# European-XFEL/xFrame

Hardware: AMD Instinct MI355X
Metric: MTIP iterations/sec, 128 q-shells x L_max=32 (higher is better)
Workload: dtype f64 (complex128); 1 GPU; BASELINE config 4: 128 shells x L_max=32, grid 128x64x128, 8 restarts per GPU on 3 streams, tutorial schedule (HIO/SW/ER, ft_stab on), fused step; restarts_per_gpu=8, restarts_total=8, streams_per_gpu=3, engines_take_turns=True, parallelism=restart-sharded x1, step_mode=fused

## Files before the change

include/mtip_hip.h:

```cpp
#ifndef MTIP_HIP_H
#define MTIP_HIP_H

#include <stdint.h>

#ifdef __cplusplus
extern "C" {
#endif

typedef struct mtip_ctx mtip_ctx;
typedef struct { double re, im; } mtip_cdouble;

enum {
    MTIP_OK = 0,
    MTIP_EINVAL = -1,
    MTIP_ENODEV = -2,
    MTIP_EHIP = -3,
    MTIP_ENOMEM = -4,
    MTIP_ESTATE = -5
};

enum { MTIP_HIO = 0, MTIP_ER = 1, MTIP_HIO_NON_FXS = 2, MTIP_ER_NON_FXS = 3 };

enum { MTIP_PRE_NONE = 0, MTIP_PRE_SQUARE = 1 , MTIP_PRE_ABS = 2  };

// ... 166 lines not shown
int mtip2d_run(mtip2d_ctx* ctx, int method, int ft_stab, int n_steps, const double* betas, double* real_err);
int mtip2d_run_async(mtip2d_ctx* ctx, int method, int ft_stab, int n_steps, const double* betas);
int mtip2d_fetch_errors(mtip2d_ctx* ctx, int64_t first_step, int64_t n_steps, double* real_err);
int mtip2d_fetch_main_errors(mtip2d_ctx* ctx, int64_t first_step, int64_t n_steps, double* main_err);
int mtip2d_fetch_reciprocal_metrics(mtip2d_ctx* ctx, int64_t first_step, int64_t n_steps, double* deg2, double* l2);
int mtip2d_shrinkwrap(mtip2d_ctx* ctx, double sigma, double threshold, double error_limit, uint8_t* enforced);
int mtip2d_refresh_reciprocal_density(mtip2d_ctx* ctx);
int mtip2d_begin_sub_loop(mtip2d_ctx* ctx);
int mtip2d_select_best(mtip2d_ctx* ctx);
int mtip2d_select_best_where(mtip2d_ctx* ctx, const uint8_t* select);
int mtip2d_get_density(mtip2d_ctx* ctx, int batch, int which, mtip_cdouble* rho);
int mtip2d_get_reciprocal_density(mtip2d_ctx* ctx, int batch, int which, mtip_cdouble* F);
int mtip2d_get_support(mtip2d_ctx* ctx, int batch, int which, uint8_t* support);
int mtip2d_get_unknowns(mtip2d_ctx* ctx, int batch, mtip_cdouble* unknowns);
int mtip2d_get_best_error(mtip2d_ctx* ctx, double* best_error, int64_t* n_steps_done);
int mtip2d_synchronize(mtip2d_ctx* ctx);

int mtip_profile(mtip_ctx* ctx, int enable);
int mtip_profile_get(mtip_ctx* ctx, const char* name, double* total_ms, int64_t* launches);
int mtip_profile_reset(mtip_ctx* ctx);
int mtip_debug_jacobi_sweeps(mtip_ctx* ctx, int32_t* out);
int mtip_debug_chain_timing(mtip_ctx* ctx, int64_t* out);
int mtip_debug_hankel_tiles(mtip_ctx* ctx, int* ct, int* n_tiles, int* n_row_blocks);
int mtip_debug_projection_slots(mtip_ctx* ctx);
#define MTIP_POLAR_TIMING_SLOTS 40
int mtip_debug_polar_timing(mtip_ctx* ctx, int64_t* out);
int mtip_debug_spin(mtip_ctx* ctx, double microseconds);
int mtip_debug_check_jacobi_schedule(mtip_ctx* ctx, int k_max);

#ifdef __cplusplus
}
#endif
#endif
```

xframe_amd/csrc/k_hankel.hip:

```cpp
#include "mtip_internal.h"
#include <vector>

void launch_hankel_mfma(mtip_ctx* c, const double2* in, double2* out, int inverse);

void launch_hankel(mtip_ctx* c, const double2* in, double2* out, int inverse) {
    ProfScope ps(c, "hankel");
    launch_hankel_mfma(c, in, out, inverse);
}

__global__ void __launch_bounds__(256) k_coeff_diff(const double2* __restrict__ a, const double2* __restrict__ b,
                                                    double2* __restrict__ out, int N, int nlm, long long total) {
    const long long idx = (long long)blockIdx.x * blockDim.x + threadIdx.x;
    if (idx >= total) return;
    const int q = (int)((idx / nlm) % N);
    double2 v = a[idx];
    if (q > 0) v = csub(v, b[idx]);
    out[idx] = v;
}

void launch_coeff_diff(mtip_ctx* c, const double2* a, const double2* b, double2* out) {
    const long long total = (long long)c->B * c->N * c->nlm;
    hipLaunchKernelGGL(k_coeff_diff, dim3((unsigned)div_up(total, 256)), dim3(256), 0, c->stream, a, b, out, c->N,
                       c->nlm, total);
}

#define HT_CT_MAX 5
#define HT_KC 16
#define HT_ROWS 128
#define HT_WS (HT_ROWS + 16)
#define HT_THREADS 512
#define HT_NW (HT_KC * HT_ROWS / HT_THREADS)

struct HankelTile32 { int l, cflat0; };

template <int HT_CT, bool SUB>
__global__ void __launch_bounds__(HT_THREADS) k_hankel_tile(const double* __restrict__ in, double* __restrict__ out,
                                                            const double* __restrict__ W,
                                                            const HankelTile32* __restrict__ tiles, int N, int Np, int L,
                                                            int B, int poffs, double scale, int sign,
                                                            const double* __restrict__ in_sub, const uint8_t* __restrict__ sub_mask) {
    constexpr int HT_COLS = 16 * HT_CT;
    constexpr int HT_XS = HT_COLS + 16;
    constexpr int HT_NX = (HT_KC * HT_COLS + HT_THREADS - 1) / HT_THREADS;
    __shared__ double Ws[2][HT_KC][HT_WS];
    __shared__ double Xs[2][HT_KC][HT_XS];
    __shared__ double Ss[SUB ? 2 : 1][SUB ? HT_KC : 1][HT_XS];
    const int tid = threadIdx.x;
    const int wave = tid >> 6, lane = tid & 63;
    const HankelTile32 tinfo = tiles[blockIdx.x];
    const int l = tinfo.l;
    const int k_base = blockIdx.y * HT_ROWS;
    const int ncl = 4 * l + 2;
    const int nlm2 = 2 * (L + 1) * (L + 1);
    const double* Wl = W + (size_t)l * Np * N;
    const int wrow = tid >> 5, wcol = (tid & 31) * 4;
    int xrow[HT_NX], xc[HT_NX];
    size_t xoff[HT_NX];
    bool xok[HT_NX], xsub[HT_NX];
#pragma unroll
    for (int j = 0; j < HT_NX; ++j) {
        const int e = tid + j * HT_THREADS;
        xrow[j] = e / HT_COLS;
        xc[j] = e - xrow[j] * HT_COLS;
        const int cflat = tinfo.cflat0 + xc[j];
        xok[j] = xrow[j] < HT_KC && cflat < B * ncl;
        const int b = xok[j] ? cflat / ncl : 0;
        const int within = xok[j] ? cflat - b * ncl : 0;
        xoff[j] = (size_t)b * N * nlm2 + 2 * (size_t)l * l + within;
        xsub[j] = SUB && (sub_mask == nullptr || sub_mask[b] != 0);
    }
    double rw0[HT_NW], rx0[HT_NX], rw1[HT_NW], rx1[HT_NX];
    double rs0[SUB ? HT_NX : 1], rs1[SUB ? HT_NX : 1];
    auto request = [&](int p0, double (&rw)[HT_NW], double (&rx)[HT_NX], double (&rs)[SUB ? HT_NX : 1]) {
        const int p = p0 + wrow;
        const bool p_ok = p < Np;
        const double* wr = Wl + (size_t)(p_ok ? p : 0) * N + k_base + wcol;
#pragma unroll
        for (int j = 0; j < HT_NW; ++j) rw[j] = (p_ok && k_base + wcol + j < N) ? wr[j] : 0.0;
#pragma unroll
        for (int j = 0; j < HT_NX; ++j) {
            const bool ok = xok[j] && p0 + xrow[j] < Np;
            const size_t o = xoff[j] + (size_t)(p0 + xrow[j] + poffs) * nlm2;
            rx[j] = ok ? in[o] : 0.0;
            if (SUB) {
                rs[j] = (ok && xsub[j]) ? in_sub[o] : 0.0;
                rx[j] -= rs[j];
            }
        }
    };
    auto deposit = [&](int buf, const double (&rw)[HT_NW], const double (&rx)[HT_NX], const double (&rs)[SUB ? HT_NX : 1]) {
#pragma unroll
        for (int j = 0; j < HT_NW; ++j) Ws[buf][wrow][wcol + j] = rw[j];
#pragma unroll
        for (int j = 0; j < HT_NX; ++j)
            if (xrow[j] < HT_KC) {
                Xs[buf][xrow[j]][xc[j]] = rx[j];
                if (SUB) Ss[buf][xrow[j]][xc[j]] = rs[j];
            }
    };
    const int li = lane & 15, kk = lane >> 4;
    v4f64 acc[HT_CT];
#pragma unroll
    for (int t = 0; t < HT_CT; ++t) acc[t] = v4f64{0.0, 0.0, 0.0, 0.0};
    auto multiply = [&](int buf) {
#pragma unroll
        for (int s = 0; s < HT_KC / 4; ++s) {
            const double af = Ws[buf][4 * s + kk][wave * 16 + li];
#pragma unroll
            for (int t = 0; t < HT_CT; ++t) {
                const double bf = Xs[buf][4 * s + kk][16 * t + li];
                acc[t] = __builtin_amdgcn_mfma_f64_16x16x4f64(af, bf, acc[t], 0, 0, 0);
            }
            if (SUB && wave == 0 && k_base == 0) {
                const double a0 = li == 0 ? af : 0.0;
#pragma unroll
                for (int t = 0; t < HT_CT; ++t) {
                    const double sf = Ss[buf][4 * s + kk][16 * t + li];
                    acc[t] = __builtin_amdgcn_mfma_f64_16x16x4f64(a0, sf, acc[t], 0, 0, 0);
                }
            }
        }
    };
    const int n_chunks = (Np + HT_KC - 1) / HT_KC;
    request(0, rw0, rx0, rs0);
    deposit(0, rw0, rx0, rs0);
    if (n_chunks > 1) request(HT_KC, rw1, rx1, rs1);
    if (n_chunks > 2) request(2 * HT_KC, rw0, rx0, rs0);
    __syncthreads();
    for (int i = 0; i < n_chunks; i += 2) {
        multiply(0);
        if (i + 1 < n_chunks) deposit(1, rw1, rx1, rs1);
        __syncthreads();
        if (i + 3 < n_chunks) request((i + 3) * HT_KC, rw1, rx1, rs1);
        if (i + 1 >= n_chunks) break;
        multiply(1);
        if (i + 2 < n_chunks) deposit(0, rw0, rx0, rs0);
        __syncthreads();
        if (i + 4 < n_chunks) request((i + 4) * HT_KC, rw0, rx0, rs0);
    }
    int r = l & 3;
    if (sign < 0) r = (4 - r) & 3;
    const bool is_im = (li & 1) != 0;
#pragma unroll
    for (int t = 0; t < HT_CT; ++t) {
        const int cflat = tinfo.cflat0 + 16 * t + li;
        const bool col_ok = cflat < B * ncl;
        const int b = col_ok ? cflat / ncl : 0;
        const int within = col_ok ? cflat - b * ncl : 0;
        const size_t col_off = (size_t)b * N * nlm2 + 2 * (size_t)l * l + within;
#pragma unroll
        for (int j = 0; j < 4; ++j) {
            double v = acc[t][j] * scale;
            const double partner = __shfl_xor(v, 1, 64);
            double o;
            if (r == 0) o = v;
            else if (r == 2) o = -v;
            else if (r == 1) o = is_im ? partner : -partner;
            else o = is_im ? -partner : partner;
            const int k = k_base + wave * 16 + kk + 4 * j;
            if (col_ok && k < N) out[col_off + (size_t)k * nlm2] = o;
        }
    }
}

bool hankel_has_difference(const mtip_ctx* c) { return c->d_htiles32 != nullptr; }

int hankel_row_blocks(const mtip_ctx* c) { return div_up(c->N, HT_ROWS); }

void launch_hankel_mfma_sub(mtip_ctx* c, const double2* in, const double2* in_sub, double2* out, int inverse, const uint8_t* sub_mask) {
    const dim3 grid((unsigned)c->n_htiles32, (unsigned)hankel_row_blocks(c));
#define HT_LAUNCH(CT, SUBF)                                                                                                  \
    hipLaunchKernelGGL((k_hankel_tile<CT, SUBF>), grid, dim3(HT_THREADS), 0, c->stream, reinterpret_cast<const double*>(in), \
                       reinterpret_cast<double*>(out), (const double*)c->d_W, (const HankelTile32*)c->d_htiles32, c->N,      \
                       c->Np, c->L, c->B, c->cfg.hankel_trapz ? 1 : 0, inverse ? c->inv_scale : c->fwd_scale,                \
                       inverse ? +1 : -1, reinterpret_cast<const double*>(in_sub), sub_mask)
    if (in_sub != nullptr) {
        switch (c->htile_ct) {
            case 1: HT_LAUNCH(1, true); break;
            case 2: HT_LAUNCH(2, true); break;
            case 3: HT_LAUNCH(3, true); break;
            default: HT_LAUNCH(5, true); break;
        }
    } else {
        switch (c->htile_ct) {
            case 1: HT_LAUNCH(1, false); break;
            case 2: HT_LAUNCH(2, false); break;
            case 3: HT_LAUNCH(3, false); break;
            default: HT_LAUNCH(5, false); break;
        }
    }
#undef HT_LAUNCH
}

void launch_hankel_mfma(mtip_ctx* c, const double2* in, double2* out, int inverse) {
    launch_hankel_mfma_sub(c, in, nullptr, out, inverse);
}

int build_hankel_tiles(mtip_ctx* c) {
    std::vector<HankelTile32> t32;
    const int cts[4] = {5, 3, 2, 1};
    for (int ci = 0; ci < 4; ++ci) {
        t32.clear();
        c->htile_ct = cts[ci];
        for (int l = c->L; l >= 0; --l) {
            const int ncols = c->B * (4 * l + 2);
            for (int c0 = 0; c0 < ncols; c0 += 16 * cts[ci]) t32.push_back(HankelTile32{l, c0});
        }
        if (c->htile_force > 0 ? cts[ci] == c->htile_force : (int)t32.size() * hankel_row_blocks(c) * 5 >= c->n_cu * 4) break;
    }
    {
        const int X = 8;
        std::vector<std::vector<HankelTile32>> q(X);
        size_t i0 = 0;
        while (i0 < t32.size()) {
            size_t i1 = i0;
// ... 26 lines not shown
```

xframe_amd/csrc/mtip_api.hip:

```cpp
#include "mtip_internal.h"
#include <algorithm>
#include <cmath>
#include <cstdlib>
#include <cstring>

static thread_local std::string g_create_error;

#define CTX_CHECK(c)                       \
    do {                                   \
        if ((c) == nullptr) return MTIP_EINVAL; \
    } while (0)
#define FAIL(c, code, msg)      \
    do {                        \
        (c)->err = (msg);       \
        return (code);          \
    } while (0)

static int post_launch(mtip_ctx* c, const char* what) {
    hipError_t e = hipGetLastError();
    if (e != hipSuccess) {
        c->err = std::string(what) + ": " + hipGetErrorString(e);
        return MTIP_EHIP;
    }
    return MTIP_OK;
// ... 87 lines not shown
    auto A = [&](int r) { if (rc == MTIP_OK) rc = r; };
    if (hipStreamCreateWithFlags(&c->stream, hipStreamNonBlocking) != hipSuccess) A(MTIP_EHIP);
    {
        int ncu = 0;
        if (hipDeviceGetAttribute(&ncu, hipDeviceAttributeMultiprocessorCount, device) == hipSuccess && ncu > 0) c->n_cu = ncu;
    }
    (void)hipEventCreate(&c->ev0);
    (void)hipEventCreate(&c->ev1);
    A(dev_alloc(c, &c->d_cost, c->nt));
    A(dev_alloc(c, &c->d_gw, c->nt));
    A(dev_alloc(c, &c->d_P, (size_t)(L + 1) * (L + 2) / 2 * c->nt));
    A(dev_alloc(c, &c->d_poff, L + 2));
    c->npairs = (L + 1) * (L + 2) / 2;
    A(dev_alloc(c, &c->d_PT, (size_t)(c->nt / 2 + 1) * c->npairs));
    A(dev_alloc(c, &c->d_AB, (size_t)c->npairs + L + 1));
    A(dev_alloc(c, &c->d_lmtab, c->npairs));
    A(dev_alloc(c, &c->d_PTc, (size_t)(c->nt / 2 + 1) * 768));
    A(dev_alloc(c, &c->d_lmc, 768));
    if (const char* e = std::getenv("MTIP_DEG2_SIMPLE")) c->deg2_simple = std::atoi(e) != 0;
    if (const char* e = std::getenv("MTIP_HANKEL_CT")) {
        const int v = std::atoi(e);
        c->htile_force = (v == 1 || v == 2 || v == 3 || v == 5) ? v : 0;
    }
    if (rc == MTIP_OK) rc = build_hankel_tiles(c);
    A(dev_alloc(c, &c->d_twN, c->np));
    A(dev_alloc(c, &c->d_tw, c->np / 2));
    A(dev_alloc(c, &c->d_r, N));
    A(dev_alloc(c, &c->d_q, N));
    A(dev_alloc(c, &c->d_W, (size_t)(L + 1) * c->Np * N));
    c->kl.assign(L + 1, 0);
    c->used.assign(L + 1, 0);
    c->active.assign(L + 1, 0);
    c->voff.assign(L + 2, 0);
    c->xoff.assign(L + 2, 0);
    c->uoff.assign(L + 2, 0);
    c->have_V.assign(L + 1, 0);
    c->v_real.assign(L + 1, 1);
    c->psw = read_proj_switches();
    for (int l = 0; l <= L; ++l) {
        const int n = 2 * l + 1, k = std::min(n, N);
        c->kl[l] = k;
        c->voff[l + 1] = c->voff[l] + N * k;
        c->xoff[l + 1] = c->xoff[l] + k * n;
        c->uoff[l + 1] = c->uoff[l] + k * k;
    }
    c->vtot = c->voff[L + 1];
// ... 1085 lines not shown
    if (!c->d_polar_dbg) {
        int r = dev_alloc(c, &c->d_polar_dbg, n);
        if (r) return r;
        MTIP_HIP_CHECK(c, hipMemsetAsync(c->d_polar_dbg, 0, n * sizeof(long long), c->stream));
    }
    if (out) MTIP_HIP_CHECK(c, mtip_copy(c, out, c->d_polar_dbg, n * sizeof(long long), hipMemcpyDeviceToHost));
    return MTIP_OK;
}

int mtip_debug_chain_timing(mtip_ctx* c, int64_t* out) {
    CTX_CHECK(c);
    (void)hipSetDevice(c->device);
    const size_t n = (size_t)3 * c->B * c->N * MTIP_CHAIN_DBG_SLOTS;
    MTIP_HIP_CHECK(c, hipStreamSynchronize(c->stream));
    if (!c->d_chain_dbg) {
        int r = dev_alloc(c, &c->d_chain_dbg, n);
        if (r) return r;
        MTIP_HIP_CHECK(c, hipMemsetAsync(c->d_chain_dbg, 0, n * sizeof(long long), c->stream));
    }
    if (out) MTIP_HIP_CHECK(c, mtip_copy(c, out, c->d_chain_dbg, n * sizeof(long long), hipMemcpyDeviceToHost));
    return MTIP_OK;
}

int mtip_debug_check_jacobi_schedule(mtip_ctx* c, int k_max) {
    CTX_CHECK(c);
    if (k_max < 2 || k_max > 127) FAIL(c, MTIP_EINVAL, "k_max must be in [2, 127]");
    (void)hipSetDevice(c->device);
    MTIP_HIP_CHECK(c, hipStreamSynchronize(c->stream));
    const int r = build_jacobi_schedule(c, k_max);
    if (r != MTIP_OK) FAIL(c, r, "pairing schedule failed its verification");
    return MTIP_OK;
}

int mtip_profile_reset(mtip_ctx* c) {
    CTX_CHECK(c);
    prof_flush(c);
    c->prof_data.clear();
    return MTIP_OK;
}

}

void prof_flush(mtip_ctx* c) {
    if (c->prof_pending.empty()) {
        c->prof_next = 0;
        return;
// ... 15 lines not shown
```

xframe_amd/csrc/mtip_internal.h:

```cpp
#pragma once
#include <hip/hip_runtime.h>
#include <stdint.h>
#include <algorithm>
#include <map>
#include <string>
#include <type_traits>
#include <utility>
#include <vector>
#include "../../include/mtip_hip.h"

#ifndef MTIP_PIN_VGPRS4
#define MTIP_PIN_VGPRS4(a, b, c, d) asm volatile("" : "+v"(a), "+v"(b), "+v"(c), "+v"(d));
#endif
#ifndef MTIP_WAIT_LDS
#define MTIP_WAIT_LDS() asm volatile("s_waitcnt lgkmcnt(0)" ::: "memory")
#endif


#ifndef MTIP_WAVE_LDS_SYNC
#define MTIP_WAVE_LDS_SYNC()                        \
    do {                                            \
        asm volatile("" ::: "memory");              \
        __builtin_amdgcn_wave_barrier();            \
        asm volatile("" ::: "memory");              \
// ... 10 lines not shown
}
__device__ __forceinline__ double2 cadd(double2 a, double2 b) { return make_double2(a.x + b.x, a.y + b.y); }
__device__ __forceinline__ double2 csub(double2 a, double2 b) { return make_double2(a.x - b.x, a.y - b.y); }
__device__ __forceinline__ double2 cscale(double2 a, double s) { return make_double2(a.x * s, a.y * s); }
__device__ __forceinline__ double cabs2(double2 a) { return a.x * a.x + a.y * a.y; }
__device__ __forceinline__ int isqrt_lm(int lm) {
    int l = (int)sqrt((double)lm);
    while (l * l > lm) --l;
    while ((l + 1) * (l + 1) <= lm) ++l;
    return l;
}
__device__ __forceinline__ double2 cmul_ipow(double2 a, int l, int sign) {
    int r = l & 3;
    if (sign < 0) r = (4 - r) & 3;
    switch (r) {
        case 0: return a;
        case 1: return make_double2(-a.y, a.x);
        case 2: return make_double2(-a.x, -a.y);
        default: return make_double2(a.y, -a.x);
    }
}

#define MTIP_CHAIN_DBG_SLOTS 18
#define MTIP_POLAR_DBG_SLOTS MTIP_POLAR_TIMING_SLOTS
enum { SL_CUR = 0, SL_OUT = 1, SL_BEST = 2, SL_SUP = 3, SL_SUP_BEST = 4, SL_ENFORCE = 5, SL_HAS_ERR = 6, SL_HIST = 7, SL_N = 8 };

enum { RC_SUPPORT = 1, RC_VALUE_LO = 2, RC_VALUE_HI = 4, RC_LIMIT_IMAG = 8 };

struct RealParams {
    uint32_t flags, hio_flags;
    double lo, hi, imag_thr;
};

__device__ __forceinline__ double2 real_update_point(const RealParams& rp, int method, double beta, double2 w, double2 pv,
                                                     bool S, double2& P_out) {
    double2 P = w;
    uint32_t viol = 0;
    if (rp.flags & RC_SUPPORT) {
        if (!S) {
            P = make_double2(0.0, 0.0);
            viol |= RC_SUPPORT;
        }
    }
    if ((rp.flags & RC_VALUE_LO) && (rp.flags & RC_VALUE_HI)) {
        if (P.x < rp.lo) { P.x = rp.lo; viol |= RC_VALUE_LO; }
        if (P.x > rp.hi) { P.x = rp.hi; viol |= RC_VALUE_LO; }
// ... 186 lines not shown
    DevBuf<int> d_lmtab;
    int npairs = 0;
    ShtPlan sht;
    DevBuf<double2> d_twN;
    DevBuf<double2> d_tw;
    DevBuf<double> d_W;
    int n_cu = 256;
    JacobiSchedule js;
    uint32_t im_which = 0;
    DevBuf<uint8_t> d_im_zmask;
    DevBuf<double2> d_im_IIref, d_im_ccdref;
    DevBuf<double> d_rl2_wr, d_rl2_wt, d_rl2_part, d_rl2_hist;
    DevBuf<double> d_im_fq;
    DevBuf<double2> d_im_part;
    DevBuf<double> d_im_qq, d_im_ccdT, d_im_P, d_im_refavg, d_im_refw, d_im_hist;
    double im_ccd_inv_norm = 0.0;
    int so_order = -1;
    DevBuf<long long> d_polar_dbg;
    DevBuf<double2> d_c0n;
    DevBuf<long long> d_chain_dbg;
    bool c0n_valid = false;
    DevBuf<HankelTile32> d_htiles32;
    int htile_force = 0;
    int n_htiles32 = 0, htile_ct = 5;
    double fwd_scale = 0, inv_scale = 0;
    bool have_angular = false, have_radial = false, have_weights = false, have_support = false, have_errw = false;
    ProjSwitches psw;
    ProjPlan pp;
    std::vector<int> kl, used, active, voff, xoff, uoff;
    DevBuf<int> d_active;
    DevBuf<int> d_sweeps;
    std::vector<char> v_real;
    std::vector<double2> h_V;
    int vr = VR_NONE;
    long long proj_calls = 0;
    DevBuf<int> d_kl, d_used, d_voff, d_xoff, d_uoff;
    int vtot = 0, xtot = 0, utot = 0;
    DevBuf<double2> d_V;
    DevBuf<uint8_t> d_rmask;
    std::vector<char> have_V;
    double n_particles = 1.0;
    int deg2_enable = 0;
    DevBuf<double2> d_Bref;
    DevBuf<double> d_Bnorm;
    DevBuf<double> d_deg2_part;
    bool deg2_simple = false;
// ... 37 lines not shown

void plan_sht(mtip_ctx* c);
int launch_sht_forward(mtip_ctx* c, const double2* grid, double2* coeff, int prologue, int in_slot = -1);
struct InvEpilogue {
    int mode = EPI_STORE;
    const double2* F = nullptr;
    const double* fixed = nullptr;
    const double* shell_scale = nullptr;
    const double2* coeff_sub = nullptr;
    RealEpi real;
    int out_slot = -1;
};
int launch_sht_inverse(mtip_ctx* c, const double2* coeff, double2* grid, const InvEpilogue& epi);
void build_legendre_tables(mtip_ctx* c, const double* cos_theta);
int sht_no_kernel(mtip_ctx* c, const char* what, int epi_mode);
void launch_sht_forward_fused(mtip_ctx* c, const double2* grid, double2* coeff, int prologue, int in_slot);
int launch_sht_inverse_fused(mtip_ctx* c, const double2* coeff, double2* grid, const InvEpilogue& epi);
void launch_sht_forward_reg(mtip_ctx* c, const double2* grid, double2* coeff, int prologue, int in_slot);
int launch_sht_inverse_reg(mtip_ctx* c, const double2* coeff, double2* grid, const InvEpilogue& epi);
int launch_sht_chain(mtip_ctx* c, const double2* coeff, double2* grid, const InvEpilogue& epi, int prologue, double2* coeff_out);
void launch_hankel(mtip_ctx* c, const double2* in, double2* out, int inverse);
bool hankel_has_difference(const mtip_ctx* c);
void launch_hankel_mfma_sub(mtip_ctx* c, const double2* in, const double2* in_sub, double2* out, int inverse, const uint8_t* sub_mask = nullptr);
int build_jacobi_schedule(mtip_ctx* c, int kmax);
int jacobi_groups(int k);
int build_hankel_tiles(mtip_ctx* c);
int hankel_row_blocks(const mtip_ctx* c);
int launch_invariant_metrics(mtip_ctx* c, const double2* Ilm, long long step);
int launch_reciprocal_l2_metric(mtip_ctx* c, const double2* F, const double2* Fp, long long step);
void launch_deg2(mtip_ctx* c, const double2* Ilm, double2* Bl);
void launch_coeff_diff(mtip_ctx* c, const double2* a, const double2* b, double2* out);
int launch_project_coefficients(mtip_ctx* c, const double2* Ilm, double2* out, bool real_intensity = false);
void plan_projection(mtip_ctx* c);
void plan_rproj(mtip_ctx* c);
void invalidate_projection(mtip_ctx* c);
int launch_rproj(mtip_ctx* c, double2* coef);
int launch_apply_unknowns(mtip_ctx* c, const double2* Ilm, double2* out);
void launch_deg2_metric(mtip_ctx* c, const double2* Ilm, double* out );
void launch_real_update(mtip_ctx* c, const double2* rho_p, const double2* prev, const double2* rho_rt, double2* out,
                        int method, double beta, int use_slots);
void launch_finish_step(mtip_ctx* c, long long step_index, int nblk = 0);
void launch_abs_to_fixed(mtip_ctx* c);
void launch_modulus_plain(mtip_ctx* c, const double2* F, const double2* Inew, double2* out);
void launch_modulus_fixed_slots(mtip_ctx* c, const double2* F);
void launch_copy_to_slot(mtip_ctx* c, const double2* src, double2* dst_slots, int which);
void launch_sw_clamp(mtip_ctx* c, const double2* conv, double* tmp_real);
// ... 91 lines not shown
```

xframe_amd/fxs/_lib.py:

```python
import ctypes as C
import os

import numpy as np

os.environ.setdefault('GPU_MAX_HW_QUEUES', '8')

_HERE = os.path.dirname(os.path.abspath(__file__))
DEFAULT_LIB = os.path.join(os.path.dirname(_HERE), 'csrc', 'libmtip_hip.so')

c_double_p = C.POINTER(C.c_double)
c_u8_p = C.POINTER(C.c_uint8)
c_void = C.c_void_p


class MtipCfg(C.Structure):
    _fields_ = [('n_radial', C.c_int32), ('l_max', C.c_int32), ('n_theta', C.c_int32), ('n_phi', C.c_int32),
                ('n_batch', C.c_int32), ('hankel_trapz', C.c_int32), ('fused', C.c_int32), ('reserved', C.c_int32)]


class MtipCorrelateCfg(C.Structure):
    _fields_ = [('n_q', C.c_int32), ('n_phi', C.c_int32), ('n_q1', C.c_int32), ('n_q2', C.c_int32), ('filter_kind', C.c_int32),
                ('roi_lo', C.c_int32), ('roi_hi', C.c_int32), ('roi_filter', C.c_int32), ('roi_normalize', C.c_int32),
                ('shared_mask', C.c_int32), ('filter_k', C.c_double), ('roi_min', C.c_double), ('roi_max', C.c_double)]

# ... 113 lines not shown
    'mtip_op_so3_find_rotation': (C.c_int, [c_void, c_void, c_void, C.c_int, C.c_int, c_void, c_void, c_void]),
    'mtip_op_rotate_coefficients_grid': (C.c_int, [c_void, c_void, c_void, c_void, c_void, c_void]),
    'mtip_op_hermitian_eig': (C.c_int, [c_void, C.c_int, C.c_int, c_void, c_void, c_void]),
    'mtip_op_symmetric_eig': (C.c_int, [c_void, C.c_int, C.c_int, c_void, c_void, c_void]),
    'mtip_op_cc_to_deg2': (C.c_int, [c_void, C.c_int, C.c_int, C.c_int, C.c_int, C.c_int, C.c_uint32, c_void, c_void, c_void, c_void, c_void]),
    'mtip_correlate_create': (c_void, [c_void, C.POINTER(MtipCorrelateCfg), c_void, c_void, c_void]),
    'mtip_correlate_destroy': (None, [c_void]),
    'mtip_correlate_add': (C.c_int, [c_void, C.c_int, c_void, c_void]),
    'mtip_correlate_num_patterns': (C.c_int, [c_void]),
    'mtip_correlate_get_partial': (C.c_int, [c_void, c_void, c_void, c_void, c_void]),
    'mtip_correlate_merge': (C.c_int, [c_void, c_void, c_void, C.c_int, c_void, c_void]),
    'mtip_correlate_finalize': (C.c_int, [c_void, C.c_int, C.c_int, C.c_int, C.c_int, C.c_int, c_void, c_void]),
    'mtip_resample_create': (c_void, [c_void, C.POINTER(MtipResampleCfg), c_void, c_void, c_void, c_void]),
    'mtip_resample_destroy': (None, [c_void]),
    'mtip_resample_run': (C.c_int, [c_void, C.c_int, c_void, C.c_int, c_void, c_void, c_void, C.POINTER(C.c_int64)]),
    'mtip_correlate_add_detector': (C.c_int, [c_void, c_void, C.c_int, c_void, C.c_int, c_void, C.POINTER(C.c_int64)]),
    'mtip_profile': (C.c_int, [c_void, C.c_int]),
    'mtip_profile_get': (C.c_int, [c_void, C.c_char_p, C.POINTER(C.c_double), C.POINTER(C.c_int64)]),
    'mtip_profile_reset': (C.c_int, [c_void]),
    'mtip_debug_jacobi_sweeps': (C.c_int, [c_void, c_void]),
    'mtip_debug_projection_slots': (C.c_int, [c_void]),
    'mtip_debug_hankel_tiles': (C.c_int, [c_void, c_void, c_void, c_void]),
    'mtip_debug_chain_timing': (C.c_int, [c_void, c_void]),
    'mtip_debug_check_jacobi_schedule': (C.c_int, [c_void, C.c_int]),
    'mtip_debug_polar_timing': (C.c_int, [c_void, c_void]),
    'mtip_debug_spin': (C.c_int, [c_void, C.c_double]),
}

EXPORTED_SYMBOLS = tuple(_SIGNATURES)
_libs = {}


def load(path=None):
    path = os.path.abspath(path or DEFAULT_LIB)
    if path in _libs:
        return _libs[path]
    if not os.path.exists(path):
        raise MtipError(f'{path} not found: build it with `python -c "import __graft_entry__ as g; g.build()"` '
                        '(hipcc --offload-arch=gfx950). There is no CPU fallback.')
    try:
        import torch
    except ImportError:
        pass
    lib = C.CDLL(path)
    for name, (res, args) in _SIGNATURES.items():
        fn = getattr(lib, name)
# ... 24 lines not shown
```

xframe_amd/fxs/engine.py:

```python
import ctypes as C

import numpy as np

from . import _lib, hostsetup as hs
from .settings import reciprocity_coefficient, resolve

METHOD_ID = {'HIO': 0, 'ER': 1, 'HIO_non_FXS': 2, 'ER_non_FXS': 3}


class Engine:
    def __init__(self, settings=None, data=None, n_batch=1, device=0, fused=True, lib_path=None,
                 n_radial=None, l_max=None, max_q=None):
        self.lib = _lib.load(lib_path)
        self.device_index = int(device)
        self.emulated = hasattr(self.lib, 'mtip_emulated')
        opt = resolve(settings)
        self.opt = opt
        g = opt['grid']
        self.N = int(n_radial if n_radial is not None else g['n_radial_points'])
        self.L = int(l_max if l_max is not None else g['max_order'])
        self.kappa = float(reciprocity_coefficient(opt['fourier_transform']))
        self.mode = opt['fourier_transform']['type']
        if max_q is None:
            max_q = g['max_q']
# ... 602 lines not shown
    def profile_get(self, name):
        ms, n = C.c_double(0), C.c_int64(0)
        self._ck(self.lib.mtip_profile_get(self.ctx, name.encode(), C.byref(ms), C.byref(n)))
        return ms.value, n.value

    def debug_spin(self, microseconds):
        self._ck(self.lib.mtip_debug_spin(self.ctx, float(microseconds)))

    def jacobi_sweeps(self):
        out = np.zeros((self.B, self.L + 1), np.int32)
        self._ck(self.lib.mtip_debug_jacobi_sweeps(self.ctx, _lib.ptr(out)))
        return out & 0xff

    def jacobi_active_columns(self):
        out = np.zeros((self.B, self.L + 1), np.int32)
        self._ck(self.lib.mtip_debug_jacobi_sweeps(self.ctx, _lib.ptr(out)))
        return (out >> 8) & 0xffff

    def hankel_tiles(self):
        ct, nt, nr = C.c_int(0), C.c_int(0), C.c_int(0)
        self._ck(self.lib.mtip_debug_hankel_tiles(self.ctx, C.byref(ct), C.byref(nt), C.byref(nr)))
        return ct.value, nt.value, nr.value

    def projection_slots(self):
        n = self.lib.mtip_debug_projection_slots(self.ctx)
        if n < 0:
            self._ck(n)
        return int(n)

    def jacobi_closing_step(self):
        out = np.zeros((self.B, self.L + 1), np.int32)
        self._ck(self.lib.mtip_debug_jacobi_sweeps(self.ctx, _lib.ptr(out)))
        return (out >> 24) & 3

    @property
    def thetas(self):
        return self.theta

    @property
    def phis(self):
        return self.phi

    def ft(self, grid):
        return self.fourier_transform(grid)[0]

    def forward_l(self, grid):
# ... 106 lines not shown
```

Before: 17180 MTIP iterations/s.

## Pipeline Hankel MFMA tiles with async global-to-LDS loads and 3-stage buffering

Rewrites the Hankel tile kernel's main loop to use global_load_lds direct DMA into a dynamically sized multi-stage LDS ring (default 3 stages), with vmcnt-based waits instead of register staging and double-buffered syncthreads. It also XOR-swizzles the X tile layout to avoid bank conflicts and replaces the extra row-0 MFMA for the difference term with a masked subtract plus a scalar FMA chain. The aim is to hide global-load latency and cut register and LDS-store traffic. The cost is more LDS per block, which may reduce occupancy, plus more complex waitcnt logic. A timed debug variant and API hook are added.

Result: faster. 17470 MTIP iterations/s (median of 6 runs) (+1.7%).

```diff
diff --git a/include/mtip_hip.h b/include/mtip_hip.h
--- a/include/mtip_hip.h
+++ b/include/mtip_hip.h
@@ -212,6 +212,7 @@
 int mtip_debug_jacobi_sweeps(mtip_ctx* ctx, int32_t* out);
 int mtip_debug_chain_timing(mtip_ctx* ctx, int64_t* out);
 int mtip_debug_hankel_tiles(mtip_ctx* ctx, int* ct, int* n_tiles, int* n_row_blocks);
+int mtip_debug_hankel_timing(mtip_ctx* ctx, int difference, int inverse, int64_t* out);
 int mtip_debug_projection_slots(mtip_ctx* ctx);
 #define MTIP_POLAR_TIMING_SLOTS 40
 int mtip_debug_polar_timing(mtip_ctx* ctx, int64_t* out);
diff --git a/xframe_amd/csrc/k_hankel.hip b/xframe_amd/csrc/k_hankel.hip
--- a/xframe_amd/csrc/k_hankel.hip
+++ b/xframe_amd/csrc/k_hankel.hip
@@ -1,4 +1,5 @@
 #include "mtip_internal.h"
+#include <type_traits>
 #include <vector>
 
 void launch_hankel_mfma(mtip_ctx* c, const double2* in, double2* out, int inverse);
@@ -30,48 +31,101 @@
 #define HT_WS (HT_ROWS + 16)
 #define HT_THREADS 512
 #define HT_NW (HT_KC * HT_ROWS / HT_THREADS)
+#ifndef HT_NS
+#define HT_NS 3
+#endif
 
 struct HankelTile32 { int l, cflat0; };
 
 template <int HT_CT, bool SUB>
+struct HankelLds {
+    static constexpr int COLS = 16 * HT_CT;
+    static constexpr int W_STAGE = HT_KC * HT_WS;
+    static constexpr int X_STAGE = HT_KC * COLS;
+    static constexpr int STAGE = W_STAGE + (SUB ? 2 : 1) * X_STAGE;
+    static constexpr size_t BYTES = (size_t)HT_NS * STAGE * sizeof(double);
+};
+
+__device__ __forceinline__ void ht_dma16(const double* src, double* dst, int lane) {
+#if defined(__HIP_DEVICE_COMPILE__)
+    (void)lane;
+    __builtin_amdgcn_global_load_lds((const __attribute__((address_space(1))) void*)src,
+                                     (__attribute__((address_space(3))) void*)dst, 16, 0, 0);
+#else
+    dst[2 * lane] = src[0];
+    dst[2 * lane + 1] = src[1];
+#endif
+}
+template <int CNT>
+__device__ __forceinline__ void ht_wait_vm() {
+#if defined(__HIP_DEVICE_COMPILE__)
+    asm volatile("s_waitcnt vmcnt(%0)" ::"n"(CNT) : "memory");
+#endif
+}
+__device__ __forceinline__ void ht_barrier() {
+#if defined(__HIP_DEVICE_COMPILE__)
+    asm volatile("s_waitcnt lgkmcnt(0)" ::: "memory");
+    __builtin_amdgcn_s_barrier();
+    asm volatile("" ::: "memory");
+#else
+    __syncthreads();
+#endif
+}
+
+template <int HT_CT, bool SUB, bool ROW0_MFMA, bool TIMED>
 __global__ void __launch_bounds__(HT_THREADS) k_hankel_tile(const double* __restrict__ in, double* __restrict__ out,
                                                             const double* __restrict__ W,
                                                             const HankelTile32* __restrict__ tiles, int N, int Np, int L,
                                                             int B, int poffs, double scale, int sign,
-                                                            const double* __restrict__ in_sub, const uint8_t* __restrict__ sub_mask) {
-    constexpr int HT_COLS = 16 * HT_CT;
-    constexpr int HT_XS = HT_COLS + 16;
+                                                            const double* __restrict__ in_sub, const uint8_t* __restrict__ sub_mask,
+                                                            long long* __restrict__ dbg) {
+    using G = HankelLds<HT_CT, SUB>;
+    constexpr int HT_COLS = G::COLS;
     constexpr int HT_NX = (HT_KC * HT_COLS + HT_THREADS - 1) / HT_THREADS;
-    __shared__ double Ws[2][HT_KC][HT_WS];
-    __shared__ double Xs[2][HT_KC][HT_XS];
-    __shared__ double Ss[SUB ? 2 : 1][SUB ? HT_KC : 1][HT_XS];
+    constexpr bool DIRECT0 = SUB && !ROW0_MFMA;
+    constexpr int NQ = 2 * HT_CT;
+    constexpr int NXI = (NQ + 7) / 8;
+    constexpr int NHI = NQ % 8;
+    constexpr int NXL = NHI ? NXI - 1 : NXI;
+    HIP_DYNAMIC_SHARED(double, lds)
     const int tid = threadIdx.x;
-    const int wave = tid >> 6, lane = tid & 63;
+    const int lane = tid & 63;
+    const int wave = __builtin_amdgcn_readfirstlane(tid >> 6);
+    long long* tl = reinterpret_cast<long long*>(lds + HT_NS * G::STAGE);
+    auto stamp = [&](int slot) {
+        if constexpr (TIMED) {
+            if (wave == 0 || wave == 5) {
+                const long long t = clock64();
+                if (lane == 0) tl[(wave ? 1 : 0) * MTIP_HANKEL_DBG_SLOTS + slot] = t;
+            }
+        }
+    };
+    auto stamp_chunk = [&](int chunk, int what) {
+        if (chunk < MTIP_HANKEL_DBG_CHUNKS) stamp(2 + 4 * chunk + what);
+    };
+    if constexpr (TIMED) {
+        if (tid < 2 * MTIP_HANKEL_DBG_SLOTS) tl[tid] = 0;
+        __syncthreads();
+        stamp(0);
+    }
     const HankelTile32 tinfo = tiles[blockIdx.x];
     const int l = tinfo.l;
     const int k_base = blockIdx.y * HT_ROWS;
     const int ncl = 4 * l + 2;
     const int nlm2 = 2 * (L + 1) * (L + 1);
+    const int ncols = B * ncl;
     const double* Wl = W + (size_t)l * Np * N;
+    auto xs_idx = [](int r, int c) { return r * HT_COLS + ((HT_COLS % 32 == 0) ? (c ^ ((r & 1) << 4)) : c); };
     const int wrow = tid >> 5, wcol = (tid & 31) * 4;
     int xrow[HT_NX], xc[HT_NX];
-    size_t xoff[HT_NX];
-    bool xok[HT_NX], xsub[HT_NX];
 #pragma unroll
     for (int j = 0; j < HT_NX; ++j) {
         const int e = tid + j * HT_THREADS;
         xrow[j] = e / HT_COLS;
         xc[j] = e - xrow[j] * HT_COLS;
-        const int cflat = tinfo.cflat0 + xc[j];
-        xok[j] = xrow[j] < HT_KC && cflat < B * ncl;
-        const int b = xok[j] ? cflat / ncl : 0;
-        const int within = xok[j] ? cflat - b * ncl : 0;
-        xoff[j] = (size_t)b * N * nlm2 + 2 * (size_t)l * l + within;
-        xsub[j] = SUB && (sub_mask == nullptr || sub_mask[b] != 0);
-    }
-    double rw0[HT_NW], rx0[HT_NX], rw1[HT_NW], rx1[HT_NX];
-    double rs0[SUB ? HT_NX : 1], rs1[SUB ? HT_NX : 1];
-    auto request = [&](int p0, double (&rw)[HT_NW], double (&rx)[HT_NX], double (&rs)[SUB ? HT_NX : 1]) {
+    }
+    double rw[HT_NW], rx[HT_NX], rs[SUB ? HT_NX : 1];
+    auto request = [&](int p0) {
         const int p = p0 + wrow;
         const bool p_ok = p < Np;
         const double* wr = Wl + (size_t)(p_ok ? p : 0) * N + k_base + wcol;
@@ -79,72 +133,205 @@
         for (int j = 0; j < HT_NW; ++j) rw[j] = (p_ok && k_base + wcol + j < N) ? wr[j] : 0.0;
 #pragma unroll
         for (int j = 0; j < HT_NX; ++j) {
-            const bool ok = xok[j] && p0 + xrow[j] < Np;
-            const size_t o = xoff[j] + (size_t)(p0 + xrow[j] + poffs) * nlm2;
+            const int cflat = tinfo.cflat0 + xc[j];
+            const bool ok = xrow[j] < HT_KC && cflat < ncols && p0 + xrow[j] < Np;
+            const int b = ok ? cflat / ncl : 0;
+            const int within = ok ? cflat - b * ncl : 0;
+            const size_t o = (size_t)b * N * nlm2 + 2 * (size_t)l * l + within + (size_t)(p0 + xrow[j] + poffs) * nlm2;
             rx[j] = ok ? in[o] : 0.0;
-            if (SUB) {
-                rs[j] = (ok && xsub[j]) ? in_sub[o] : 0.0;
-                rx[j] -= rs[j];
-            }
+            if (SUB) rs[j] = (ok && (sub_mask == nullptr || sub_mask[b] != 0)) ? in_sub[o] : 0.0;
         }
     };
-    auto deposit = [&](int buf, const double (&rw)[HT_NW], const double (&rx)[HT_NX], const double (&rs)[SUB ? HT_NX : 1]) {
-#pragma unroll
-        for (int j = 0; j < HT_NW; ++j) Ws[buf][wrow][wcol + j] = rw[j];
+    auto deposit = [&](int st) {
+        double* ws = lds + st * G::STAGE;
+#pragma unroll
+        for (int j = 0; j < HT_NW; ++j) ws[wrow * HT_WS + wcol + j] = rw[j];
 #pragma unroll
         for (int j = 0; j < HT_NX; ++j)
             if (xrow[j] < HT_KC) {
-                Xs[buf][xrow[j]][xc[j]] = rx[j];
-                if (SUB) Ss[buf][xrow[j]][xc[j]] = rs[j];
+                ws[G::W_STAGE + xs_idx(xrow[j], xc[j])] = rx[j];
+                if (SUB) ws[G::W_STAGE + G::X_STAGE + xs_idx(xrow[j], xc[j])] = rs[j];
             }
     };
     const int li = lane & 15, kk = lane >> 4;
+    bool subf[HT_CT];
+#pragma unroll
+    for (int t = 0; t < HT_CT; ++t) {
+        const int cflat = tinfo.cflat0 + 16 * t + li;
+        const bool ok = SUB && cflat < ncols;
+        subf[t] = ok && (sub_mask == nullptr || sub_mask[ok ? cflat / ncl : 0] != 0);
+    }
+    int subm[HT_CT];
+#pragma unroll
+    for (int t = 0; t < HT_CT; ++t) subm[t] = subf[t] ? -1 : 0;
     v4f64 acc[HT_CT];
 #pragma unroll
     for (int t = 0; t < HT_CT; ++t) acc[t] = v4f64{0.0, 0.0, 0.0, 0.0};
-    auto multiply = [&](int buf) {
+    bool tile_sub = SUB && sub_mask == nullptr;
+    if (SUB && sub_mask != nullptr) {
+        const int c_last = (tinfo.cflat0 + HT_COLS < ncols ? tinfo.cflat0 + HT_COLS : ncols) - 1;
+        for (int b = tinfo.cflat0 / ncl; b <= c_last / ncl; ++b) tile_sub = tile_sub || sub_mask[b] != 0;
+    }
+    const bool row0 = SUB && k_base == 0 && tile_sub;
+    constexpr int NW0 = (HT_COLS + 63) / 64;
+    const int c0 = tid < HT_COLS ? tid : 0;
+    double chain0 = 0.0;
+    auto multiply = [&](int st) {
+        const double* ws = lds + st * G::STAGE;
+        const double* xs = ws + G::W_STAGE;
+        const double* ss = xs + G::X_STAGE;
 #pragma unroll
         for (int s = 0; s < HT_KC / 4; ++s) {
-            const double af = Ws[buf][4 * s + kk][wave * 16 + li];
+            const double af = ws[(4 * s + kk) * HT_WS + wave * 16 + li];
+            double sv[SUB ? HT_CT : 1];
 #pragma unroll
             for (int t = 0; t < HT_CT; ++t) {
-                const double bf = Xs[buf][4 * s + kk][16 * t + li];
+                double bf = xs[xs_idx(4 * s + kk, 16 * t + li)];
+                if (SUB) {
+                    const double sraw = ss[xs_idx(4 * s + kk, 16 * t + li)];
+                    sv[t] = __hiloint2double(__double2hiint(sraw) & subm[t], __double2loint(sraw) & subm[t]);
+                    bf -= sv[t];
+                }
                 acc[t] = __builtin_amdgcn_mfma_f64_16x16x4f64(af, bf, acc[t], 0, 0, 0);
             }
-            if (SUB && wave == 0 && k_base == 0) {
+            if (SUB && ROW0_MFMA && wave == 0 && k_base == 0) {
                 const double a0 = li == 0 ? af : 0.0;
 #pragma unroll
-                for (int t = 0; t < HT_CT; ++t) {
-                    const double sf = Ss[buf][4 * s + kk][16 * t + li];
-                    acc[t] = __builtin_amdgcn_mfma_f64_16x16x4f64(a0, sf, acc[t], 0, 0, 0);
+                for (int t = 0; t < HT_CT; ++t) acc[t] = __builtin_amdgcn_mfma_f64_16x16x4f64(a0, sv[t], acc[t], 0, 0, 0);
+            }
+        }
+        if (DIRECT0 && row0 && wave < NW0) {
+#pragma unroll
+            for (int s = 0; s < HT_KC / 4; ++s) {
+                double w0[4], s0[4];
+#pragma unroll
+                for (int k = 0; k < 4; ++k) {
+                    w0[k] = ws[(4 * s + k) * HT_WS];
+                    s0[k] = ss[xs_idx(4 * s + k, c0)];
+                    chain0 = fma(w0[k], xs[xs_idx(4 * s + k, c0)] - s0[k], chain0);
                 }
+#pragma unroll
+                for (int k = 0; k < 4; ++k) chain0 = fma(w0[k], s0[k], chain0);
             }
         }
     };
     const int n_chunks = (Np + HT_KC - 1) / HT_KC;
-    request(0, rw0, rx0, rs0);
-    deposit(0, rw0, rx0, rs0);
-    if (n_chunks > 1) request(HT_KC, rw1, rx1, rs1);
-    if (n_chunks > 2) request(2 * HT_KC, rw0, rx0, rs0);
-    __syncthreads();
-    for (int i = 0; i < n_chunks; i += 2) {
-        multiply(0);
-        if (i + 1 < n_chunks) deposit(1, rw1, rx1, rs1);
+    if (k_base + HT_ROWS <= N && (N & 1) == 0) {
+        const int n_full = Np / HT_KC;
+        const double* wp = Wl + (size_t)(2 * wave) * N + k_base + 2 * lane;
+        const double* xp[NXI];
+        const double* sp[SUB ? NXI : 1];
+#pragma unroll
+        for (int jj = 0; jj < NXI; ++jj) {
+            const int g = (wave + 8 * jj) * 64 + lane;
+            const int r = g / (8 * HT_CT);
+            int c = 2 * (g - r * 8 * HT_CT);
+            if (HT_COLS % 32 == 0) c ^= (r & 1) << 4;
+            int cflat = tinfo.cflat0 + c;
+            if (cflat >= ncols) cflat = tinfo.cflat0;
+            const int b = cflat / ncl;
+            const size_t o = (size_t)b * N * nlm2 + 2 * (size_t)l * l + (cflat - b * ncl) + (size_t)((r & (HT_KC - 1)) + poffs) * nlm2;
+            xp[jj] = in + o;
+            if (SUB) sp[jj] = in_sub + o;
+        }
+        const size_t wstep = (size_t)HT_KC * N, xstep = (size_t)HT_KC * nlm2;
+        auto issue = [&](int st) {
+            double* ws = lds + st * G::STAGE;
+            ht_dma16(wp, ws + (2 * wave) * HT_WS, lane);
+            ht_dma16(wp + N, ws + (2 * wave + 1) * HT_WS, lane);
+            wp += wstep;
+#pragma unroll
+            for (int jj = 0; jj < NXI; ++jj)
+                if (wave + 8 * jj < NQ) {
+                    ht_dma16(xp[jj], ws + G::W_STAGE + (wave + 8 * jj) * 128, lane);
+                    xp[jj] += xstep;
+                    if (SUB && tile_sub) {
+                        ht_dma16(sp[jj], ws + G::W_STAGE + G::X_STAGE + (wave + 8 * jj) * 128, lane);
+                        sp[jj] += xstep;
+                    }
+                }
+        };
+        const bool hi = NHI == 0 || wave < NHI;
+        auto wait_behind = [&](auto k) {
+            constexpr int K = decltype(k)::value;
+            if (SUB && tile_sub) { if (hi) ht_wait_vm<K * (2 + 2 * NXI)>(); else ht_wait_vm<K * (2 + 2 * NXL)>(); }
+            else { if (hi) ht_wait_vm<K * (2 + NXI)>(); else ht_wait_vm<K * (2 + NXL)>(); }
+        };
+        int st_in = 0, st_out = 0;
+        auto next = [](int st) { return st + 1 == HT_NS ? 0 : st + 1; };
+        for (int i = 0; i < HT_NS - 1 && i < n_full; ++i) {
+            issue(st_in);
+            st_in = next(st_in);
+        }
+        stamp(1);
+        int i = 0;
+        for (; i + HT_NS - 1 < n_full; ++i) {
+            stamp_chunk(i, 0);
+            wait_behind(std::integral_constant<int, HT_NS - 2>());
+            stamp_chunk(i, 1);
+            ht_barrier();
+            stamp_chunk(i, 2);
+            issue(st_in);
+            st_in = next(st_in);
+            multiply(st_out);
+            st_out = next(st_out);
+            stamp_chunk(i, 3);
+        }
+        for (; i < n_full; ++i) {
+            const int pending = n_full - 1 - i;
+            stamp_chunk(i, 0);
+            if (HT_NS > 3 && pending >= 2) wait_behind(std::integral_constant<int, 2>());
+            else if (pending == 1) wait_behind(std::integral_constant<int, 1>());
+            else ht_wait_vm<0>();
+            stamp_chunk(i, 1);
+            ht_barrier();
+            stamp_chunk(i, 2);
+            multiply(st_out);
+            st_out = next(st_out);
+            stamp_chunk(i, 3);
+        }
+        if (n_full < n_chunks) {
+            request(n_full * HT_KC);
+            stamp_chunk(n_full, 0);
+            deposit(st_out);
+            stamp_chunk(n_full, 1);
+            __syncthreads();
+            stamp_chunk(n_full, 2);
+            multiply(st_out);
+            stamp_chunk(n_full, 3);
+        }
+    } else {
+        request(0);
+        stamp(1);
+        for (int i = 0; i < n_chunks; ++i) {
+            stamp_chunk(i, 0);
+            deposit(i & 1);
+            stamp_chunk(i, 1);
+            __syncthreads();
+            stamp_chunk(i, 2);
+            if (i + 1 < n_chunks) request((i + 1) * HT_KC);
+            multiply(i & 1);
+            stamp_chunk(i, 3);
+        }
+    }
+    if (DIRECT0 && row0) {
         __syncthreads();
-        if (i + 3 < n_chunks) request((i + 3) * HT_KC, rw1, rx1, rs1);
-        if (i + 1 >= n_chunks) break;
-        multiply(1);
-        if (i + 2 < n_chunks) deposit(0, rw0, rx0, rs0);
+        if (tid < HT_COLS) lds[tid] = chain0;
         __syncthreads();
-        if (i + 4 < n_chunks) request((i + 4) * HT_KC, rw0, rx0, rs0);
-    }
+        if (wave == 0 && kk == 0) {
+#pragma unroll
+            for (int t = 0; t < HT_CT; ++t)
+                if (subf[t]) acc[t][0] = lds[16 * t + li];
+        }
+    }
+    stamp(MTIP_HANKEL_DBG_SLOTS - 2);
     int r = l & 3;
     if (sign < 0) r = (4 - r) & 3;
     const bool is_im = (li & 1) != 0;
 #pragma unroll
     for (int t = 0; t < HT_CT; ++t) {
         const int cflat = tinfo.cflat0 + 16 * t + li;
-        const bool col_ok = cflat < B * ncl;
+        const bool col_ok = cflat < ncols;
         const int b = col_ok ? cflat / ncl : 0;
         const int within = col_ok ? cflat - b * ncl : 0;
         const size_t col_off = (size_t)b * N * nlm2 + 2 * (size_t)l * l + within;
@@ -161,36 +348,54 @@
             if (col_ok && k < N) out[col_off + (size_t)k * nlm2] = o;
         }
     }
+    if constexpr (TIMED) {
+        stamp(MTIP_HANKEL_DBG_SLOTS - 1);
+        __syncthreads();
+        if (tid < 2 * MTIP_HANKEL_DBG_SLOTS)
+            dbg[((size_t)blockIdx.y * gridDim.x + blockIdx.x) * 2 * MTIP_HANKEL_DBG_SLOTS + tid] = tl[tid];
+    }
 }
 
 bool hankel_has_difference(const mtip_ctx* c) { return c->d_htiles32 != nullptr; }
 
 int hankel_row_blocks(const mtip_ctx* c) { return div_up(c->N, HT_ROWS); }
 
+#define HT_LAUNCH(CT, SUBF, ROW0, TIMEDF, DBG)                                                                               \
+    hipLaunchKernelGGL((k_hankel_tile<CT, SUBF, ROW0, TIMEDF>), grid, dim3(HT_THREADS),                                      \
+                       (HankelLds<CT, SUBF>::BYTES + (TIMEDF ? 2 * MTIP_HANKEL_DBG_SLOTS * sizeof(long long) : 0)),          \
+                       c->stream, reinterpret_cast<const double*>(in), reinterpret_cast<double*>(out),                       \
+                       (const double*)c->d_W, (const HankelTile32*)c->d_htiles32, c->N, c->Np, c->L, c->B,                   \
+                       c->cfg.hankel_trapz ? 1 : 0, inverse ? c->inv_scale : c->fwd_scale, inverse ? +1 : -1,                \
+                       reinterpret_cast<const double*>(in_sub), sub_mask, DBG)
+#define HT_LAUNCH_CT(SUBF, ROW0, TIMEDF, DBG)                   \
+    switch (c->htile_ct) {                                      \
+        case 1: HT_LAUNCH(1, SUBF, ROW0, TIMEDF, DBG); break;   \
+        case 2: HT_LAUNCH(2, SUBF, ROW0, TIMEDF, DBG); break;   \
+        case 3: HT_LAUNCH(3, SUBF, ROW0, TIMEDF, DBG); break;   \
+        default: HT_LAUNCH(5, SUBF, ROW0, TIMEDF, DBG); break;  \
+    }
 void launch_hankel_mfma_sub(mtip_ctx* c, const double2* in, const double2* in_sub, double2* out, int inverse, const uint8_t* sub_mask) {
     const dim3 grid((unsigned)c->n_htiles32, (unsigned)hankel_row_blocks(c));
-#define HT_LAUNCH(CT, SUBF)                                                                                                  \
-    hipLaunchKernelGGL((k_hankel_tile<CT, SUBF>), grid, dim3(HT_THREADS), 0, c->stream, reinterpret_cast<const double*>(in), \
-                       reinterpret_cast<double*>(out), (const double*)c->d_W, (const HankelTile32*)c->d_htiles32, c->N,      \
-                       c->Np, c->L, c->B, c->cfg.hankel_trapz ? 1 : 0, inverse ? c->inv_scale : c->fwd_scale,                \
-                       inverse ? +1 : -1, reinterpret_cast<const double*>(in_sub), sub_mask)
+    if (in_sub != nullptr && c->hankel_row0_mfma) {
+        HT_LAUNCH_CT(true, true, false, nullptr)
+    } else if (in_sub != nullptr) {
+        HT_LAUNCH_CT(true, false, false, nullptr)
+    } else {
+        HT_LAUNCH_CT(false, false, false, nullptr)
+    }
+}
+
+void launch_hankel_timed(mtip_ctx* c, const double2* in, const double2* in_sub, double2* out, int inverse, long long* dbg) {
+    const dim3 grid((unsigned)c->n_htiles32, (unsigned)hankel_row_blocks(c));
+    const uint8_t* sub_mask = nullptr;
     if (in_sub != nullptr) {
-        switch (c->htile_ct) {
-            case 1: HT_LAUNCH(1, true); break;
-            case 2: HT_LAUNCH(2, true); break;
-            case 3: HT_LAUNCH(3, true); break;
-            default: HT_LAUNCH(5, true); break;
-        }
+        HT_LAUNCH_CT(true, false, true, dbg)
     } else {
-        switch (c->htile_ct) {
-            case 1: HT_LAUNCH(1, false); break;
-            case 2: HT_LAUNCH(2, false); break;
-            case 3: HT_LAUNCH(3, false); break;
-            default: HT_LAUNCH(5, false); break;
-        }
-    }
+        HT_LAUNCH_CT(false, false, true, dbg)
+    }
+}
+#undef HT_LAUNCH_CT
 #undef HT_LAUNCH
-}
 
 void launch_hankel_mfma(mtip_ctx* c, const double2* in, double2* out, int inverse) {
     launch_hankel_mfma_sub(c, in, nullptr, out, inverse);
diff --git a/xframe_amd/csrc/mtip_api.hip b/xframe_amd/csrc/mtip_api.hip
--- a/xframe_amd/csrc/mtip_api.hip
+++ b/xframe_amd/csrc/mtip_api.hip
@@ -133,6 +133,7 @@
         const int v = std::atoi(e);
         c->htile_force = (v == 1 || v == 2 || v == 3 || v == 5) ? v : 0;
     }
+    if (const char* e = std::getenv("MTIP_HANKEL_ROW0_MFMA")) c->hankel_row0_mfma = std::atoi(e) != 0;
     if (rc == MTIP_OK) rc = build_hankel_tiles(c);
     A(dev_alloc(c, &c->d_twN, c->np));
     A(dev_alloc(c, &c->d_tw, c->np / 2));
@@ -1264,6 +1265,22 @@
     return MTIP_OK;
 }
 
+int mtip_debug_hankel_timing(mtip_ctx* c, int difference, int inverse, int64_t* out) {
+    CTX_CHECK(c);
+    if (!c->have_weights) FAIL(c, MTIP_ESTATE, "mtip_set_hankel_weights has not been called");
+    if (!out) FAIL(c, MTIP_EINVAL, "null buffer");
+    (void)hipSetDevice(c->device);
+    SYNC();
+    const size_t n = (size_t)c->n_htiles32 * hankel_row_blocks(c) * 2 * MTIP_HANKEL_DBG_SLOTS;
+    DevBuf<long long> d_dbg;
+    if (d_dbg.alloc(n) != hipSuccess) FAIL(c, MTIP_ENOMEM, "hipMalloc failed");
+    MTIP_HIP_CHECK(c, hipMemsetAsync(d_dbg, 0, n * sizeof(long long), c->stream));
+    launch_hankel_timed(c, c->d_c[0], difference ? (const double2*)c->d_c[1] : nullptr, c->d_c[2], inverse ? 1 : 0, d_dbg);
+    SYNC();
+    D2H(out, d_dbg, n * sizeof(long long));
+    return post_launch(c, "mtip_debug_hankel_timing");
+}
+
 int mtip_debug_check_jacobi_schedule(mtip_ctx* c, int k_max) {
     CTX_CHECK(c);
     if (k_max < 2 || k_max > 127) FAIL(c, MTIP_EINVAL, "k_max must be in [2, 127]");
diff --git a/xframe_amd/csrc/mtip_internal.h b/xframe_amd/csrc/mtip_internal.h
--- a/xframe_amd/csrc/mtip_internal.h
+++ b/xframe_amd/csrc/mtip_internal.h
@@ -56,6 +56,8 @@
 }
 
 #define MTIP_CHAIN_DBG_SLOTS 18
+#define MTIP_HANKEL_DBG_CHUNKS 10
+#define MTIP_HANKEL_DBG_SLOTS (2 + 4 * MTIP_HANKEL_DBG_CHUNKS + 2)
 #define MTIP_POLAR_DBG_SLOTS MTIP_POLAR_TIMING_SLOTS
 enum { SL_CUR = 0, SL_OUT = 1, SL_BEST = 2, SL_SUP = 3, SL_SUP_BEST = 4, SL_ENFORCE = 5, SL_HAS_ERR = 6, SL_HIST = 7, SL_N = 8 };
 
@@ -288,6 +290,7 @@
     bool c0n_valid = false;
     DevBuf<HankelTile32> d_htiles32;
     int htile_force = 0;
+    bool hankel_row0_mfma = false;
     int n_htiles32 = 0, htile_ct = 5;
     double fwd_scale = 0, inv_scale = 0;
     bool have_angular = false, have_radial = false, have_weights = false, have_support = false, have_errw = false;
@@ -371,6 +374,8 @@
 void launch_hankel(mtip_ctx* c, const double2* in, double2* out, int inverse);
 bool hankel_has_difference(const mtip_ctx* c);
 void launch_hankel_mfma_sub(mtip_ctx* c, const double2* in, const double2* in_sub, double2* out, int inverse, const uint8_t* sub_mask = nullptr);
+void launch_hankel_timed(mtip_ctx* c, const double2* in, const double2* in_sub, double2* out, int inverse, long long* dbg);
+int hankel_row_blocks(const mtip_ctx* c);
 int build_jacobi_schedule(mtip_ctx* c, int kmax);
 int jacobi_groups(int k);
 int build_hankel_tiles(mtip_ctx* c);
diff --git a/xframe_amd/fxs/_lib.py b/xframe_amd/fxs/_lib.py
--- a/xframe_amd/fxs/_lib.py
+++ b/xframe_amd/fxs/_lib.py
@@ -159,6 +159,7 @@
     'mtip_debug_projection_slots': (C.c_int, [c_void]),
     'mtip_debug_hankel_tiles': (C.c_int, [c_void, c_void, c_void, c_void]),
     'mtip_debug_chain_timing': (C.c_int, [c_void, c_void]),
+    'mtip_debug_hankel_timing': (C.c_int, [c_void, C.c_int, C.c_int, c_void]),
     'mtip_debug_check_jacobi_schedule': (C.c_int, [c_void, C.c_int]),
     'mtip_debug_polar_timing': (C.c_int, [c_void, c_void]),
     'mtip_debug_spin': (C.c_int, [c_void, C.c_double]),
diff --git a/xframe_amd/fxs/engine.py b/xframe_amd/fxs/engine.py
--- a/xframe_amd/fxs/engine.py
+++ b/xframe_amd/fxs/engine.py
@@ -648,6 +648,14 @@
         self._ck(self.lib.mtip_debug_hankel_tiles(self.ctx, C.byref(ct), C.byref(nt), C.byref(nr)))
         return ct.value, nt.value, nr.value
 
+    HANKEL_DBG_SLOTS = 44
+
+    def hankel_timing(self, difference=False, inverse=False):
+        _, nt, nr = self.hankel_tiles()
+        out = np.zeros((nt * nr, 2, self.HANKEL_DBG_SLOTS), np.int64)
+        self._ck(self.lib.mtip_debug_hankel_timing(self.ctx, int(difference), int(inverse), _lib.ptr(out)))
+        return out
+
     def projection_slots(self):
         n = self.lib.mtip_debug_projection_slots(self.ctx)
         if n < 0:
```
